# ZhonghuaYi/FocusFlow_official

Measured on AMD Instinct MI355X. Metric: frame-pairs/sec FF-RAFT 384x512 iters=12, higher is better.
Workload: dtype f32 via fp16x3 split operands on the f16 MFMA pipe (f32 accumulate, fp32-level accuracy); 1 GPU; FF-RAFT forward (test_mode), 8 pairs/GPU 384x512, iters=12, fp32 correlation pyramid, random-init weights, ORB-like masks (BASELINE configs[1]); pairs_per_gpu=8, corr_pyramid=fp32, conv_precision=f16x3, hipgraph=False, skip_unused_upsample=False, parallelism=dp1 (independent shards, no collective)

## Files before the change

focusflow_official_amd/csrc/conv_small.hip:

```cpp
#include "ff_common.h"

namespace {

typedef float f32x4 __attribute__((ext_vector_type(4)));
constexpr int RUN = 8;

struct SArgs {
    FFConvParams p;
    int Cin, runs_x;
};

__device__ __forceinline__ float dot4(const f32x4 a, const f32x4 b, float acc) {
    acc = fmaf(a[0], b[0], acc); acc = fmaf(a[1], b[1], acc); acc = fmaf(a[2], b[2], acc); return fmaf(a[3], b[3], acc);
}

template <int COUT>
__global__ __launch_bounds__(256) void conv_small_kernel(const SArgs a) {
    const FFConvParams& p = a.p;
    const int lane = threadIdx.x & 63;
    const long long task = (long long)blockIdx.x * 4 + (threadIdx.x >> 6);
    const long long ntask = (long long)p.B * p.H * a.runs_x;
    if (task >= ntask) return;
    const int run = (int)(task % a.runs_x);
    const int y = (int)((task / a.runs_x) % p.H);
    const int b = (int)(task / ((long long)a.runs_x * p.H));
    const int x0 = run * RUN;
    const int H = p.H, W = p.W, K = 9 * a.Cin;

    float mine[COUT];
#pragma unroll
    for (int c = 0; c < COUT; ++c) mine[c] = 0.f;

    for (int cbase = 0; cbase < a.Cin; cbase += 256) {
        const int cpos = cbase + lane * 4;
        const bool cok = cpos < a.Cin;
        const float* xp = p.x[0];
        int ld = p.x_ld[0], cs = 0;
        if (cok) {
            const int c0 = p.x_c[0], c01 = p.x_c[0] + p.x_c[1];
            cs = cpos;
            if (cs < c0) { xp = p.x[0]; ld = p.x_ld[0]; }
            else if (cs < c01) { xp = p.x[1]; ld = p.x_ld[1]; cs -= c0; }
            else { xp = p.x[2]; ld = p.x_ld[2]; cs -= c01; }
        }
        f32x4 w[COUT][9];
#pragma unroll
        for (int c = 0; c < COUT; ++c)
#pragma unroll
            for (int t = 0; t < 9; ++t)
                w[c][t] = cok ? *reinterpret_cast<const f32x4*>(p.w + (long long)c * K + t * a.Cin + cpos) : (f32x4){0.f, 0.f, 0.f, 0.f};
        auto load = [&](int yy, int xx) {
            const bool ok = cok && (unsigned)yy < (unsigned)H && (unsigned)xx < (unsigned)W;
            const int yc = min(max(yy, 0), H - 1), xc = min(max(xx, 0), W - 1);
            const f32x4 v = *reinterpret_cast<const f32x4*>(xp + ((long long)(b * H + yc) * W + xc) * ld + cs);
            return ok ? v : (f32x4){0.f, 0.f, 0.f, 0.f};
        };
        f32x4 col[3][3];
#pragma unroll
        for (int dy = 0; dy < 3; ++dy) { col[0][dy] = load(y - 1 + dy, x0 - 1); col[1][dy] = load(y - 1 + dy, x0); }
#pragma unroll
        for (int i = 0; i < RUN; ++i) {
#pragma unroll
            for (int dy = 0; dy < 3; ++dy) col[(i + 2) % 3][dy] = load(y - 1 + dy, x0 + i + 1);
#pragma unroll
            for (int c = 0; c < COUT; ++c) {
                float s = 0.f;
#pragma unroll
                for (int dy = 0; dy < 3; ++dy)
#pragma unroll
                    for (int dx = 0; dx < 3; ++dx) s = dot4(col[(i + dx) % 3][dy], w[c][dy * 3 + dx], s);
#pragma unroll
                for (int o = 32; o > 0; o >>= 1) s += __shfl_xor(s, o);
                if (lane == i) mine[c] += s;
            }
        }
    }
    const int x = x0 + lane;
    if (lane < RUN && x < W) {
        const long long m = ((long long)b * H + y) * W + x;
#pragma unroll
        for (int c = 0; c < COUT; ++c) {
            float v = mine[c] + (p.bias ? p.bias[c] : 0.f);
            v *= p.out_scale;
            if (p.ch_scale) v = v * p.ch_scale[c] + p.ch_shift[c];
            v = ff::apply_act(v, p.act);
            if (p.res) v = ff::apply_act(v + p.res[m * p.res_ld + c], p.act_res);
            p.y[m * p.y_ld + c] = v;
            mine[c] = v;
        }
        if constexpr (COUT == 2) {
            if (p.ep_mode == FF_EP_COORDS) {
                float* c1 = const_cast<float*>(p.ep_a) + m * 2;
                const float cx = __fadd_rn(c1[0], mine[0]), cy = __fadd_rn(c1[1], mine[1]);
                c1[0] = cx;
                c1[1] = cy;
                *reinterpret_cast<f32x4*>(const_cast<float*>(p.ep_b) + m * 4) = (f32x4){__fsub_rn(cx, (float)x), __fsub_rn(cy, (float)y), 0.f, 0.f};
            }
        }
    }
}

}

namespace ff {
int conv2d_fwd_small(const FFConvParams& p, int cin, hipStream_t s) {
    const int dlh = p.dil_h ? p.dil_h : 1, dlw = p.dil_w ? p.dil_w : 1;
    if (p.w_format != FF_W_F32 || p.Cout > 2 || p.KH != 3 || p.KW != 3 || p.stride != 1 || p.pad_h != 1 || p.pad_w != 1 ||
        dlh != 1 || dlw != 1 || p.groups != 1)
        return 1;
    SArgs a;
    a.p = p;
    a.Cin = cin;
    a.runs_x = (p.W + RUN - 1) / RUN;
    const long long tasks = (long long)p.B * p.H * a.runs_x;
    const unsigned blocks = (unsigned)((tasks + 3) / 4);
    if (p.Cout == 1) conv_small_kernel<1><<<blocks, 256, 0, s>>>(a);
    else conv_small_kernel<2><<<blocks, 256, 0, s>>>(a);
    return check_launch("ff_conv2d_fwd(small)");
}
}

namespace {

struct DArgs {
    const float* x; int x_ld;
    const float* w;
    const float* bias;
    float* y; int y_ld;
    int B, H, W, Cin, runs_x;
};

template <int COUT>
__global__ __launch_bounds__(256) void deconv4x4s2_small_kernel(const DArgs a) {
    const int lane = threadIdx.x & 63;
    const int Ho = 2 * a.H, Wo = 2 * a.W;
    const long long task = (long long)blockIdx.x * 4 + (threadIdx.x >> 6);
    if (task >= (long long)a.B * Ho * a.runs_x) return;
    const int run = (int)(task % a.runs_x);
    const int oy = (int)((task / a.runs_x) % Ho);
    const int b = (int)(task / ((long long)a.runs_x * Ho));
    const int ox0 = run * RUN, n0 = ox0 >> 1;
    const int a0 = oy & 1;
    const int iy0 = (oy - 2 + a0) >> 1;
    const int K = 16 * a.Cin;

    float mine[COUT];
#pragma unroll
    for (int c = 0; c < COUT; ++c) mine[c] = 0.f;
    for (int cbase = 0; cbase < a.Cin; cbase += 256) {
        const int cpos = cbase + lane * 4;
        const bool cok = cpos < a.Cin;
        f32x4 w[COUT][2][4];
#pragma unroll
        for (int c = 0; c < COUT; ++c)
#pragma unroll
            for (int r = 0; r < 2; ++r)
#pragma unroll
                for (int bb = 0; bb < 4; ++bb)
                    w[c][r][bb] = cok ? *reinterpret_cast<const f32x4*>(a.w + (long long)c * K + ((a0 + 2 * r) * 4 + bb) * a.Cin + cpos)
                                      : (f32x4){0.f, 0.f, 0.f, 0.f};
        auto load = [&](int iy, int ix) {
            const bool ok = cok && (unsigned)iy < (unsigned)a.H && (unsigned)ix < (unsigned)a.W;
            const int yc = min(max(iy, 0), a.H - 1), xc = min(max(ix, 0), a.W - 1);
            const f32x4 v = *reinterpret_cast<const f32x4*>(a.x + ((long long)(b * a.H + yc) * a.W + xc) * a.x_ld + (cok ? cpos : 0));
            return ok ? v : (f32x4){0.f, 0.f, 0.f, 0.f};
        };
        f32x4 col[6][2];
#pragma unroll
        for (int j = 0; j < 6; ++j)
#pragma unroll
            for (int r = 0; r < 2; ++r) col[j][r] = load(iy0 + r, n0 - 1 + j);
#pragma unroll
        for (int i = 0; i < RUN; ++i) {
            const int b0 = i & 1, j0 = ((i - 2 + b0) >> 1) + 1;
#pragma unroll
            for (int c = 0; c < COUT; ++c) {
                float s = 0.f;
#pragma unroll
                for (int r = 0; r < 2; ++r)
#pragma unroll
                    for (int t = 0; t < 2; ++t) s = dot4(col[j0 + t][r], w[c][r][b0 + 2 * t], s);
#pragma unroll
                for (int o = 32; o > 0; o >>= 1) s += __shfl_xor(s, o);
                if (lane == i) mine[c] += s;
            }
        }
    }
    const int ox = ox0 + lane;
    if (lane < RUN && ox < Wo) {
        const long long m = ((long long)b * Ho + oy) * Wo + ox;
#pragma unroll
        for (int c = 0; c < COUT; ++c) a.y[m * a.y_ld + c] = mine[c] + (a.bias ? a.bias[c] : 0.f);
    }
}

}

extern "C" int ff_deconv4x4s2_small(const float* x, int x_ld, int B, int H, int W, int Cin, const float* w, const float* bias,
                                    int Cout, float* y, int y_ld, void* stream) {
    FF_REQUIRE(x && w && y && B > 0 && H > 0 && W > 0 && Cin > 0 && Cin % 4 == 0 && (Cout == 1 || Cout == 2),
               "ff_deconv4x4s2_small: Cin must be a multiple of 4, Cout 1 or 2");
    FF_REQUIRE(x_ld >= Cin && x_ld % 4 == 0 && y_ld >= Cout && ff::aligned16(x) && ff::aligned16(w), "ff_deconv4x4s2_small: ld/alignment");
    DArgs a;
    a.x = x; a.x_ld = x_ld; a.w = w; a.bias = bias; a.y = y; a.y_ld = y_ld;
    a.B = B; a.H = H; a.W = W; a.Cin = Cin;
    a.runs_x = (2 * W + RUN - 1) / RUN;
    const long long tasks = (long long)B * 2 * H * a.runs_x;
    const unsigned blocks = (unsigned)((tasks + 3) / 4);
    hipStream_t s = static_cast<hipStream_t>(stream);
    if (Cout == 1) deconv4x4s2_small_kernel<1><<<blocks, 256, 0, s>>>(a);
    else deconv4x4s2_small_kernel<2><<<blocks, 256, 0, s>>>(a);
    return ff::check_launch("ff_deconv4x4s2_small");
}
```

Before: 620.8 frame-pairs/s.

## Tile small-Cout 3x3 conv into multi-row strips with rolling row reuse and reduce-scatter

The small-Cout 3x3 conv kernel now has each wavefront compute a strip of several output rows by several columns instead of one row run of 8. Input rows are loaded once into a rolling double buffer and reused across the three vertical taps, and per-row partial sums go through a butterfly reduce-scatter rather than a full wave reduction for every output pixel. Bounds checks become bitmask selects on clamped loads. The kernel gains more register pressure (now launch_bounds 256,2), a different store layout with a lane shuffle for the coords epilogue, and a default of rows=3 with strip width 8 for Cout=1 and 4 for Cout=2.

```diff
diff --git a/focusflow_official_amd/csrc/conv_small.hip b/focusflow_official_amd/csrc/conv_small.hip
--- a/focusflow_official_amd/csrc/conv_small.hip
+++ b/focusflow_official_amd/csrc/conv_small.hip
@@ -3,33 +3,60 @@
 namespace {
 
 typedef float f32x4 __attribute__((ext_vector_type(4)));
+typedef unsigned u32x4 __attribute__((ext_vector_type(4)));
 constexpr int RUN = 8;
+constexpr int SMALL_RMAX = 8;
 
 struct SArgs {
     FFConvParams p;
-    int Cin, runs_x;
+    int Cin, rows, strips_x, strips_y;
 };
 
 __device__ __forceinline__ float dot4(const f32x4 a, const f32x4 b, float acc) {
     acc = fmaf(a[0], b[0], acc); acc = fmaf(a[1], b[1], acc); acc = fmaf(a[2], b[2], acc); return fmaf(a[3], b[3], acc);
 }
-
-template <int COUT>
-__global__ __launch_bounds__(256) void conv_small_kernel(const SArgs a) {
+__device__ __forceinline__ f32x4 keep_if(const f32x4 v, bool keep) {
+    return __builtin_bit_cast(f32x4, __builtin_bit_cast(u32x4, v) & (keep ? ~0u : 0u));
+}
+
+template <int N>
+__device__ __forceinline__ float reduce_scatter(float (&v)[N], int lane) {
+    int o = 32;
+#pragma unroll
+    for (int n = N / 2; n >= 1; n >>= 1, o >>= 1) {
+        const bool hi = lane & o;
+#pragma unroll
+        for (int j = 0; j < n; ++j) {
+            const float keep = hi ? v[j + n] : v[j], send = hi ? v[j] : v[j + n];
+            v[j] = keep + __shfl_xor(send, o);
+        }
+    }
+    float s = v[0];
+#pragma unroll
+    for (int q = 0; q < 6; ++q)
+        if ((32 >> q) <= o) s += __shfl_xor(s, 32 >> q);
+    return s;
+}
+
+template <int COUT, int SW>
+__global__ __launch_bounds__(256, 2) void conv_small_kernel(const SArgs a) {
+    constexpr int N = SW * COUT, LOW = N == 16 ? 2 : N == 8 ? 3 : 4;
+    static_assert(N == 16 || N == 8 || N == 4, "reduce_scatter: 4, 8 or 16 values per row");
     const FFConvParams& p = a.p;
     const int lane = threadIdx.x & 63;
     const long long task = (long long)blockIdx.x * 4 + (threadIdx.x >> 6);
-    const long long ntask = (long long)p.B * p.H * a.runs_x;
+    const long long ntask = (long long)p.B * a.strips_y * a.strips_x;
     if (task >= ntask) return;
-    const int run = (int)(task % a.runs_x);
-    const int y = (int)((task / a.runs_x) % p.H);
-    const int b = (int)(task / ((long long)a.runs_x * p.H));
-    const int x0 = run * RUN;
+    const int sx = (int)(task % a.strips_x);
+    const int sy = (int)((task / a.strips_x) % a.strips_y);
+    const int b = (int)(task / ((long long)a.strips_x * a.strips_y));
+    const int R = a.rows;
+    const int x0 = __builtin_amdgcn_readfirstlane(sx * SW), y0 = __builtin_amdgcn_readfirstlane(sy * R);
     const int H = p.H, W = p.W, K = 9 * a.Cin;
 
-    float mine[COUT];
-#pragma unroll
-    for (int c = 0; c < COUT; ++c) mine[c] = 0.f;
+    float mine[SMALL_RMAX];
+#pragma unroll
+    for (int r = 0; r < SMALL_RMAX; ++r) mine[r] = 0.f;
 
     for (int cbase = 0; cbase < a.Cin; cbase += 256) {
         const int cpos = cbase + lane * 4;
@@ -48,56 +75,98 @@
         for (int c = 0; c < COUT; ++c)
 #pragma unroll
             for (int t = 0; t < 9; ++t)
-                w[c][t] = cok ? *reinterpret_cast<const f32x4*>(p.w + (long long)c * K + t * a.Cin + cpos) : (f32x4){0.f, 0.f, 0.f, 0.f};
-        auto load = [&](int yy, int xx) {
-            const bool ok = cok && (unsigned)yy < (unsigned)H && (unsigned)xx < (unsigned)W;
-            const int yc = min(max(yy, 0), H - 1), xc = min(max(xx, 0), W - 1);
-            const f32x4 v = *reinterpret_cast<const f32x4*>(xp + ((long long)(b * H + yc) * W + xc) * ld + cs);
-            return ok ? v : (f32x4){0.f, 0.f, 0.f, 0.f};
+                w[c][t] = keep_if(*reinterpret_cast<const f32x4*>(p.w + (long long)c * K + t * a.Cin + (cok ? cpos : 0)), cok);
+        const float* lp = xp + (long long)b * H * W * ld + cs;
+        auto load_row = [&](f32x4 (&row)[SW + 2], int yy) {
+            const float* rp = lp + (long long)min(max(yy, 0), H - 1) * W * ld;
+#pragma unroll
+            for (int j = 0; j < SW + 2; ++j)
+                row[j] = *reinterpret_cast<const f32x4*>(rp + (long long)min(max(x0 - 1 + j, 0), W - 1) * ld);
         };
-        f32x4 col[3][3];
-#pragma unroll
-        for (int dy = 0; dy < 3; ++dy) { col[0][dy] = load(y - 1 + dy, x0 - 1); col[1][dy] = load(y - 1 + dy, x0); }
-#pragma unroll
-        for (int i = 0; i < RUN; ++i) {
-#pragma unroll
-            for (int dy = 0; dy < 3; ++dy) col[(i + 2) % 3][dy] = load(y - 1 + dy, x0 + i + 1);
-#pragma unroll
-            for (int c = 0; c < COUT; ++c) {
-                float s = 0.f;
-#pragma unroll
-                for (int dy = 0; dy < 3; ++dy)
-#pragma unroll
-                    for (int dx = 0; dx < 3; ++dx) s = dot4(col[(i + dx) % 3][dy], w[c][dy * 3 + dx], s);
-#pragma unroll
-                for (int o = 32; o > 0; o >>= 1) s += __shfl_xor(s, o);
-                if (lane == i) mine[c] += s;
+        float acc[3][COUT][SW];
+#pragma unroll
+        for (int q = 0; q < 3; ++q)
+#pragma unroll
+            for (int c = 0; c < COUT; ++c)
+#pragma unroll
+                for (int i = 0; i < SW; ++i) acc[q][c][i] = 0.f;
+        auto step = [&](f32x4 (&cur)[SW + 2], f32x4 (&nxt)[SW + 2], int k) {
+            load_row(nxt, y0 + k);
+            const bool yok = cok && (unsigned)(y0 - 1 + k) < (unsigned)H;
+#pragma unroll
+            for (int j = 0; j < SW + 2; ++j) cur[j] = keep_if(cur[j], yok && (unsigned)(x0 - 1 + j) < (unsigned)W);
+#pragma unroll
+            for (int dy = 0; dy < 3; ++dy)
+                if (k - dy >= 0 && k - dy < R) {
+#pragma unroll
+                    for (int c = 0; c < COUT; ++c)
+#pragma unroll
+                        for (int i = 0; i < SW; ++i)
+#pragma unroll
+                            for (int dx = 0; dx < 3; ++dx) acc[2 - dy][c][i] = dot4(cur[i + dx], w[c][dy * 3 + dx], acc[2 - dy][c][i]);
+                }
+            if (k >= 2) {
+                float v[N];
+#pragma unroll
+                for (int c = 0; c < COUT; ++c)
+#pragma unroll
+                    for (int i = 0; i < SW; ++i) v[c * SW + i] = acc[0][c][i];
+                const float s = reduce_scatter<N>(v, lane);
+#pragma unroll
+                for (int r = 0; r < SMALL_RMAX; ++r) mine[r] = r == k - 2 ? mine[r] + s : mine[r];
             }
-        }
-    }
-    const int x = x0 + lane;
-    if (lane < RUN && x < W) {
+#pragma unroll
+            for (int c = 0; c < COUT; ++c)
+#pragma unroll
+                for (int i = 0; i < SW; ++i) { acc[0][c][i] = acc[1][c][i]; acc[1][c][i] = acc[2][c][i]; acc[2][c][i] = 0.f; }
+        };
+        f32x4 ra[SW + 2], rb[SW + 2];
+        load_row(ra, y0 - 1);
+#pragma unroll 1
+        for (int k = 0; k < R + 2; k += 2) {
+            step(ra, rb, k);
+            if (k + 1 < R + 2) step(rb, ra, k + 1);
+        }
+    }
+    const int n = lane >> LOW, c = n / SW, x = x0 + n % SW;
+    const bool coords = COUT == 2 && p.ep_mode == FF_EP_COORDS;
+#pragma unroll
+    for (int r = 0; r < SMALL_RMAX; ++r) {
+        if (r >= R) break;
+        const int y = y0 + r;
+        const bool valid = x < W && y < H;
         const long long m = ((long long)b * H + y) * W + x;
-#pragma unroll
-        for (int c = 0; c < COUT; ++c) {
-            float v = mine[c] + (p.bias ? p.bias[c] : 0.f);
+        float v = 0.f;
+        if (valid) {
+            v = mine[r] + (p.bias ? p.bias[c] : 0.f);
             v *= p.out_scale;
             if (p.ch_scale) v = v * p.ch_scale[c] + p.ch_shift[c];
             v = ff::apply_act(v, p.act);
             if (p.res) v = ff::apply_act(v + p.res[m * p.res_ld + c], p.act_res);
+        }
+        float other = 0.f;
+        if (coords) other = __shfl_xor(v, 32);
+        if (valid && (lane & ((1 << LOW) - 1)) == 0) {
             p.y[m * p.y_ld + c] = v;
-            mine[c] = v;
-        }
-        if constexpr (COUT == 2) {
-            if (p.ep_mode == FF_EP_COORDS) {
+            if (coords && c == 0) {
                 float* c1 = const_cast<float*>(p.ep_a) + m * 2;
-                const float cx = __fadd_rn(c1[0], mine[0]), cy = __fadd_rn(c1[1], mine[1]);
+                const float cx = __fadd_rn(c1[0], v), cy = __fadd_rn(c1[1], other);
                 c1[0] = cx;
                 c1[1] = cy;
                 *reinterpret_cast<f32x4*>(const_cast<float*>(p.ep_b) + m * 4) = (f32x4){__fsub_rn(cx, (float)x), __fsub_rn(cy, (float)y), 0.f, 0.f};
             }
         }
     }
+}
+
+template <int COUT, int SW>
+int launch_small(SArgs& a, hipStream_t s) {
+    const FFConvParams& p = a.p;
+    a.strips_x = (p.W + SW - 1) / SW;
+    a.strips_y = (p.H + a.rows - 1) / a.rows;
+    const long long tasks = (long long)p.B * a.strips_y * a.strips_x;
+    conv_small_kernel<COUT, SW><<<(unsigned)((tasks + 3) / 4), 256, 0, s>>>(a);
+    return ff::check_launch("ff_conv2d_fwd(small)");
 }
 
 }
@@ -111,12 +180,16 @@
     SArgs a;
     a.p = p;
     a.Cin = cin;
-    a.runs_x = (p.W + RUN - 1) / RUN;
-    const long long tasks = (long long)p.B * p.H * a.runs_x;
-    const unsigned blocks = (unsigned)((tasks + 3) / 4);
-    if (p.Cout == 1) conv_small_kernel<1><<<blocks, 256, 0, s>>>(a);
-    else conv_small_kernel<2><<<blocks, 256, 0, s>>>(a);
-    return check_launch("ff_conv2d_fwd(small)");
+    a.rows = 3;
+#ifdef FF_LAB
+    if (const char* e = ff::tune_env("FF_SMALL_STRIP")) {
+        const int v = atoi(e);
+        a.rows = std::min(std::max(v / 10, 1), SMALL_RMAX);
+        if (v % 10 == 4) return p.Cout == 1 ? launch_small<1, 4>(a, s) : launch_small<2, 4>(a, s);
+        return p.Cout == 1 ? launch_small<1, 8>(a, s) : launch_small<2, 8>(a, s);
+    }
+#endif
+    return p.Cout == 1 ? launch_small<1, 8>(a, s) : launch_small<2, 4>(a, s);
 }
 }
 
```

Result: no change. 626.5 frame-pairs/s (median of 6 runs) (+0.9%).
